# NVIDIA/RAD-MMM

Hardware: AMD Instinct MI355X
Metric: mel-frames/sec training step (fwd+bwd) (higher is better)
Workload: dtype f32 (f16 hi.hi product + fp8 e4m3 cross terms, fp32 accumulate); 1 GPU; RADTTS flow decoder (configs/RADTTS_model_config.yaml: 8 flows, WN 1024x4, D=1048) fwd+NLL+bwd; batch_per_gpu=32, n_mel=80, frames=800, global_batch=32, parallelism=dp1, includes_optimizer=False

## Files before the change

include/radmmm_hip.h:

```cpp
#ifndef RADMMM_HIP_H
#define RADMMM_HIP_H

#include <stdint.h>

#ifdef __cplusplus
extern "C" {
#endif

#define RADMMM_ABI_VERSION 4

typedef void* radmmm_stream_t;

const char* radmmm_last_error(void);
int radmmm_abi_version(void);

enum { RADMMM_ACT_NONE = 0, RADMMM_ACT_SOFTPLUS = 1, RADMMM_ACT_RELU = 2, RADMMM_ACT_LEAKY = 3 };
enum { RADMMM_SCALE_TANH = 0, RADMMM_SCALE_EXP = 1, RADMMM_SCALE_SIGMOID = 2, RADMMM_SCALE_TRANSLATE = 3 };

#define RADMMM_SPLIT_F16 0
#define RADMMM_SPLIT_X8A 1
#define RADMMM_SPLIT_X8B 2
typedef struct { int fmt; int x8_exp; int32_t* sat_flag;
                 void* lo16;
} radmmm_split_opts;
// ... 71 lines not shown
#define RADMMM_F32_FAMILY_WGRAD16 5
#define RADMMM_F32_KERNEL_CODE(family, bl, mt, rows) ((family) * 1000000 + (bl) * 100000 + (mt) * 1000 + (rows))
int radmmm_rowgemm_f32_plan(const radmmm_rowgemm_desc* d);
int radmmm_wgrad_f32_plan(const radmmm_wgrad_desc* d);

int radmmm_weightnorm_fwd(const float* v, const float* g, float* W, float* inv_norm,
                          int Cout, int Cin, int taps, int ldw,
                          int perm_split, int off_lo, int off_hi, radmmm_stream_t stream);
int radmmm_weightnorm_bwd(const float* v, const float* g, const float* inv_norm,
                          const float* dW, int splits, int64_t split_stride,
                          float* dv, float* dg,
                          int Cout, int Cin, int taps, int ldw,
                          int perm_split, int off_lo, int off_hi,
                          const float* poison ,
                          radmmm_stream_t stream);

int radmmm_wn_input_fwd(const float* ctx, int ldctx, const float* z, int ldz,
                        float* X0 , int ldx0, int rows, int D, int h,
                        void* X0h, void* X0l ,
                        const radmmm_split_opts* so, radmmm_stream_t stream);
int radmmm_wn_input_bwd(const float* gX0, int ldx0, float* gctx, int ldctx, int ctx_accum,
                        float* gz, int ldz, int rows, int D, int h, radmmm_stream_t stream);

int radmmm_squeeze_rows(const float* in , float* out, int B, int C, int T, int g, int ld, int col0,
                        radmmm_stream_t stream);
int radmmm_unsqueeze_rows(const float* gout, float* gin , int B, int C, int T, int g, int ld, int col0,
                          radmmm_stream_t stream);

int radmmm_affine_coupling_fwd(const float* O, int ldo, const float* z, int ldz,
                               float* zout, float* log_s, int rows, int h, int scaling,
// ... 144 lines not shown
int radmmm_wgrad_rm8(const void* GYh, const void* GYx, int ldg, int g8_exp, const void* Xh, const void* Xx, int ldx, int x8_exp,
                     int R, int T, const int32_t* lens, int x_mask, float* P, int ldp, int64_t split_stride, int Mc, int Nc,
                     int taps, int dil, int splits, float acc_scale, radmmm_stream_t stream);

int radmmm_wgrad_rmh(const void* GYh, int ldg, const void* Xh, int ldx, int R, int T, const int32_t* lens, int x_mask, float* P,
                     int ldp, int64_t split_stride, int Mc, int Nc, int taps, int dil, int splits, float acc_scale,
                     radmmm_stream_t stream);

int radmmm_wgrad_rmh_shift(const void* GYh, int ldg, int g_col0, const void* Xh, int ldx, int x_col0, int shift0, int R, int T,
                           const int32_t* lens, int x_mask, float* P, int ldp, int64_t split_stride, int Mc, int Nc, int taps,
                           int dil, int splits, float acc_scale, radmmm_stream_t stream);
int radmmm_wgrad_rm_shift(const void* GYh, const void* GYl, int ldg, int g_col0, const void* Xh, const void* Xl, int ldx, int x_col0,
                          int shift0, int R, int T, const int32_t* lens, int x_mask, float* P, int ldp, int64_t split_stride,
                          int Mc, int Nc, int taps, int dil, int splits, float acc_scale, radmmm_stream_t stream);

int radmmm_split_f16_groups(const float* x, int ld, void* hi, void* lo, int ldh, int rows, int gcols, int groups, int gpitch,
                            float scale, int* sat_flag, radmmm_stream_t stream);

int64_t radmmm_lstm_scratch_bytes(int B, int H, int which);
int64_t radmmm_lstm_hseq_bytes(int B, int T, int H);
int radmmm_lstm_fwd(float* G, const float* W_hh, float* y, float* c, const int32_t* lens, void* wsplit, void* hsplit,
                    void* hseq, int B, int T, int H, radmmm_stream_t stream);
int radmmm_lstm_bwd(float* G, const float* c, const float* dy, const float* W_hh, const int32_t* lens, void* wtpack,
                    float* P, float* dcbuf, int B, int T, int H, const float* gscale, radmmm_stream_t stream);
int radmmm_lstm_last_path(int which);

int radmmm_lu_weight_fwd(const float* P, const float* lower, const float* lower_diag, const float* upper,
                         const float* upper_diag, int c, float* W, int ldw, int col_offset, float* logdet,
                         radmmm_stream_t stream);
int radmmm_lu_weight_bwd(const float* P, const float* lower, const float* lower_diag, const float* upper,
// ... 135 lines not shown
```

rad_mmm_amd/_lib.py:

```python
from __future__ import annotations

import ctypes as C
import os
from typing import Optional

import torch

_HERE = os.path.dirname(os.path.abspath(__file__))
LIB_PATH = os.environ.get("RADMMM_LIB_PATH") or os.path.join(_HERE, "libradmmm_hip.so")



def debug_env(name: str, default: Optional[str] = None) -> Optional[str]:
    if os.environ.get("RADMMM_DEBUG", "0") in ("", "0"):
        return default
    return os.environ.get(name, default)


ACT_NONE, ACT_SOFTPLUS, ACT_RELU, ACT_LEAKY = 0, 1, 2, 3
SCALE = {"tanh": 0, "exp": 1, "sigmoid": 2, "translate": 3}
ACT = {"none": 0, "softplus": 1, "relu": 2, "leaky_relu": 3}


class RadmmmError(RuntimeError):
# ... 24 lines not shown
        ("split_fmt", C.c_int), ("ch_x8_exp", C.c_int), ("c2h_x8_exp", C.c_int),
        ("sat_flag", C.c_void_p),
        ("Clo", C.c_void_p),
        ("colsum_out", C.c_void_p), ("colsum_scratch", C.c_void_p),
        ("dact_h", C.c_void_p), ("dact_x", C.c_void_p), ("lddact_h", C.c_int), ("dact_x8_exp", C.c_int),
        ("c2_src", C.c_void_p * 3), ("n_c2_src", C.c_int),
    ]


class CsItem(C.Structure):
    _fields_ = [("part", C.c_void_p), ("out", C.c_void_p), ("nparts", C.c_int), ("cols", C.c_int)]


class DactItem(C.Structure):
    _fields_ = [("saved", C.c_void_p), ("yh", C.c_void_p), ("yl", C.c_void_p), ("ylo16", C.c_void_p), ("part", C.c_void_p)]


class SplitOpts(C.Structure):
    _fields_ = [("fmt", C.c_int), ("x8_exp", C.c_int), ("sat_flag", C.c_void_p), ("lo16", C.c_void_p)]


SPLIT_F16, SPLIT_X8A, SPLIT_X8B = 0, 1, 2


def split_opts(fmt: int = 0, x8_exp: int = 0, sat_flag: Optional[torch.Tensor] = None, lo16: Optional[torch.Tensor] = None):
    return C.byref(SplitOpts(fmt, x8_exp, sat_flag.data_ptr() if sat_flag is not None else None,
                             lo16.data_ptr() if lo16 is not None else None))


class RowGemmH3Desc(C.Structure):
# ... 65 lines not shown
        "radmmm_masked_reduce": [p, i, i, i, i64, i64, i64, p, i, p, p, p],
        "radmmm_masked_reduce_bwd": [p, i, i, i, i64, i64, i64, p, i, p, p, p],
        "radmmm_fused_add_tanh_sigmoid_multiply": [p, p, i, p, i, i, i, p],
        "radmmm_film_fwd": [p, i, p, i, p, i, p, p, p, p, p, i, i, i, i, p],
        "radmmm_film_bwd": [p, i, p, i, p, i, p, p, p, p, f, i, p, p, i, p, i, p, i, p, p, p, i, i, i, p],
        "radmmm_film_bwd_sums": [p, i, p, i, p, i, p, p, p, p, p, p, p, i, i, p],
        "radmmm_film_bwd_apply": [p, i, p, i, p, i, p, p, p, p, f, i, p, p, i, p, i, p, i, p, i, i, p],
        "radmmm_split_f16": [p, i, p, p, i, i, i, f, so, p],
        "radmmm_transpose_split_act": [p, i, i, i, i, i, i, p, i, f, p, p, p, p, i, p],
        "radmmm_wgrad_h3_tiles": [i, i, i],
        "radmmm_wgrad_rm_tiles": [i, i, i],
        "radmmm_wgrad_rm": [p, p, i, p, p, i, i, i, p, i, p, i, i64, i, i, i, i, i, f, p],
        "radmmm_wgrad_rm8": [p, p, i, i, p, p, i, i, i, i, p, i, p, i, i64, i, i, i, i, i, f, p],
        "radmmm_wgrad_rmh": [p, i, p, i, i, i, p, i, p, i, i64, i, i, i, i, i, f, p],
        "radmmm_wgrad_rmh_shift": [p, i, i, p, i, i, i, i, i, p, i, p, i, i64, i, i, i, i, i, f, p],
        "radmmm_wgrad_rm_shift": [p, p, i, i, p, p, i, i, i, i, i, p, i, p, i, i64, i, i, i, i, i, f, p],
        "radmmm_split_f16_groups": [p, i, p, p, i, i, i, i, i, f, p, p],
        "radmmm_betabinom_prior": [i, i, C.c_double, p, p],
        "radmmm_prior_zoom_batch": [p, i, p, i, i, p],
        "radmmm_energy_average": [p, p, i, i, i, i, p],
        "radmmm_lu_weight_fwd": [p, p, p, p, p, i, p, i, i, p, p],
        "radmmm_lu_weight_bwd": [p, p, p, p, p, i, p, i, i, p, p, p, p, p],
        "radmmm_instnorm_fwd": [p, i, p, p, p, i, p, p, p, i, i, i, f, i, p],
        "radmmm_instnorm_bwd": [p, i, p, i, p, i, p, p, p, p, i, p, p, p, i, i, i, i, p],
        "radmmm_pq_spline_inv": [p, i, p, i, p, i, i, i, i, p],
        "radmmm_sumsq": [p, i64, p, p],
        "radmmm_radam_step": [p, p, p, p, i64, p, f, f, f, f, f, i, p],
        "radmmm_transpose_split_act_colsum": [p, i, i, i, i, i, i, p, i, f, p, p, p, p, i, p, i, i, i, p],
        "radmmm_colsum_final": [p, p, i, i, p],
        "radmmm_colsum_final_multi": [C.POINTER(CsItem), i, p], "radmmm_rowgemm_h3_colsum_rows": [C.POINTER(RowGemmH3Desc)],
# ... 258 lines not shown
```

rad_mmm_amd/csrc/elementwise.hip:

```cpp
#include <math.h>
#include <stdlib.h>

#include "common.h"
#include "split_pack.h"

namespace {

using radmmm::block_sum;
using radmmm::wave_sum;

__device__ __forceinline__ int perm_col(int ci, int perm_split, int off_lo, int off_hi) {
  return ci < perm_split ? ci + off_lo : ci - perm_split + off_hi;
}

__global__ __launch_bounds__(256) void weightnorm_fwd_kernel(
    const float* __restrict__ v, const float* __restrict__ g, float* __restrict__ W,
    float* __restrict__ inv_norm, int Cout, int Cin, int taps, int ldw, int perm_split,
    int off_lo, int off_hi) {
  __shared__ float sh[17];
  const int co = blockIdx.x;
  const int n = Cin * taps;
  const float* vr = v + (long long)co * n;
  float ss = 0.f;
  for (int i = threadIdx.x; i < n; i += blockDim.x) ss = fmaf(vr[i], vr[i], ss);
// ... 77 lines not shown
  if (threadIdx.x == 0) dg[co] = dot * inv + (poison ? poison[0] : 0.f);
  const float a = gg * inv, b = gg * dot * inv * inv * inv;
  if (VEC && n % 4 == 0) {
    for (int i = threadIdx.x * 4; i < n; i += blockDim.x * 4) {
      const float4 vv = *reinterpret_cast<const float4*>(vr + i);
      const float4 gv = *reinterpret_cast<const float4*>(gw + i);
      *reinterpret_cast<float4*>(dv + (long long)co * n + i) =
          make_float4(a * gv.x - b * vv.x, a * gv.y - b * vv.y, a * gv.z - b * vv.z, a * gv.w - b * vv.w);
    }
  } else {
    for (int i = threadIdx.x; i < n; i += blockDim.x) dv[(long long)co * n + i] = a * gw[i] - b * vr[i];
  }
}

template <int TAPS>
__global__ __launch_bounds__(256) void weightnorm_bwd_reg_kernel(
    const float* __restrict__ v, const float* __restrict__ g, const float* __restrict__ inv_norm,
    const float* __restrict__ dW, int splits, long long split_stride, float* __restrict__ dv,
    float* __restrict__ dg, int Cout, int Cin, int ldw, int perm_split, int off_lo, int off_hi,
    const float* __restrict__ poison) {
  __shared__ float sh[17];
  const int co = blockIdx.x;
  const long long n = (long long)Cin * TAPS;
  const float inv = inv_norm[co], gg = g[co], pz = poison ? poison[0] : 0.f;
  constexpr int MAXJ = 2;
  float4 vv[MAXJ][TAPS], gs[MAXJ][TAPS];
  float dot = 0.f;
#pragma unroll
  for (int j = 0; j < MAXJ; ++j) {
    const int ci = threadIdx.x * 4 + j * 1024;
    const bool on = ci < Cin;
    const int cic = on ? ci : 0;
    const int col = perm_col(cic, perm_split, off_lo, off_hi);
    const float* vp = v + (long long)co * n + (long long)cic * TAPS;
#pragma unroll
    for (int k = 0; k < TAPS; ++k) vv[j][k] = on ? *reinterpret_cast<const float4*>(vp + 4 * k) : make_float4(0.f, 0.f, 0.f, 0.f);
#pragma unroll
// ... 23 lines not shown
  const float a = gg * inv, b = gg * dot * inv * inv * inv;
#pragma unroll
  for (int j = 0; j < MAXJ; ++j) {
    const int ci = threadIdx.x * 4 + j * 1024;
    if (ci < Cin) {
      float o[4 * TAPS];
#pragma unroll
      for (int c = 0; c < 4; ++c)
#pragma unroll
        for (int k = 0; k < TAPS; ++k) o[c * TAPS + k] = a * chan_of(gs[j][k], c) - b * run_at(vv[j], c * TAPS + k);
      float* dp = dv + (long long)co * n + (long long)ci * TAPS;
#pragma unroll
      for (int k = 0; k < TAPS; ++k) *reinterpret_cast<float4*>(dp + 4 * k) = make_float4(o[4 * k], o[4 * k + 1], o[4 * k + 2], o[4 * k + 3]);
    }
  }
}

__global__ __launch_bounds__(256) void wn_input_fwd_kernel(
    const float* __restrict__ ctx, int ldctx, const float* __restrict__ z, int ldz,
    float* __restrict__ X0, int ldx0, int rows, int D, int h, _Float16* __restrict__ Xh,
    _Float16* __restrict__ Xl, int fmt, float x8_mul, void* __restrict__ lo16) {
  const long long total = (long long)rows * ldx0;
  for (long long i = blockIdx.x * (long long)blockDim.x + threadIdx.x; i < total;
       i += (long long)gridDim.x * blockDim.x) {
    const int r = (int)(i / ldx0), c = (int)(i - (long long)r * ldx0);
    float v = 0.f;
    if (c < D) v = ctx[(long long)r * ldctx + c];
    else if (c < D + h) v = z[(long long)r * ldz + (c - D)];
    if (X0) X0[i] = v;
    if (Xh) radmmm::store_split1_fmt(Xh, Xl, (long long)r * ldx0, c, fmt, x8_mul, 1.f, v, lo16);
// ... 381 lines not shown
                           (long long)split_stride, dv, dg, Cout, Cin, ldw, perm_split, off_lo, off_hi, poison);
    } else if (vec)
      hipLaunchKernelGGL(weightnorm_bwd_lds_kernel<true>, dim3(Cout), dim3(256), lds, ST(stream), v, g, inv_norm, dW,
                         splits, (long long)split_stride, dv, dg, Cout, Cin, taps, ldw, perm_split, off_lo, off_hi, poison);
    else
      hipLaunchKernelGGL(weightnorm_bwd_lds_kernel<false>, dim3(Cout), dim3(256), lds, ST(stream), v, g, inv_norm, dW,
                         splits, (long long)split_stride, dv, dg, Cout, Cin, taps, ldw, perm_split, off_lo, off_hi, poison);
  } else {
    hipLaunchKernelGGL(weightnorm_bwd_kernel, dim3(Cout), dim3(256), 0, ST(stream), v, g, inv_norm, dW,
                       splits, (long long)split_stride, dv, dg, Cout, Cin, taps, ldw, perm_split,
                       off_lo, off_hi, poison);
  }
  return radmmm::check_launch("weightnorm_bwd");
}

extern "C" int radmmm_wn_input_fwd(const float* ctx, int ldctx, const float* z, int ldz, float* X0,
                                   int ldx0, int rows, int D, int h, void* Xh, void* Xl,
                                   const radmmm_split_opts* so, radmmm_stream_t stream) {
  RADMMM_REQUIRE(ctx && z && (X0 || Xh), "wn_input_fwd: null pointer (X0 may be NULL when the split copy Xh / Xl is written)");
  RADMMM_REQUIRE(rows > 0 && D > 0 && h > 0 && ldx0 >= D + h && ldctx >= D && ldz >= h, "wn_input_fwd: bad dims");
  const int fmt = so ? so->fmt : RADMMM_SPLIT_F16;
  RADMMM_REQUIRE(fmt == RADMMM_SPLIT_F16 || !Xh || (ldx0 % 32 == 0 && abs(so->x8_exp) <= 16), "wn_input_fwd: 8-bit format needs ldx0 %% 32 == 0");
  auto a16 = [](const void* q) { return (reinterpret_cast<uintptr_t>(q) & 15) == 0; };
  auto a8 = [](const void* q) { return (reinterpret_cast<uintptr_t>(q) & 7) == 0; };
  if (D % 4 == 0 && ldctx % 4 == 0 && ldz % 4 == 0 && ldx0 % 4 == 0 && a16(ctx) && a16(z) && a16(X0) &&
      a8(Xh) && a8(Xl) && a8(so ? so->lo16 : nullptr)) {
    hipLaunchKernelGGL(wn_input_fwd4_kernel, dim3(grid_for((long long)rows * (ldx0 / 4))), dim3(256), 0, ST(stream), ctx,
                       ldctx, z, ldz, X0, ldx0, rows, D, h, static_cast<_Float16*>(Xh), static_cast<_Float16*>(Xl), fmt,
                       ldexpf(1.f, so ? so->x8_exp : 0), so ? so->lo16 : nullptr);
    return radmmm::check_launch("wn_input_fwd");
// ... 245 lines not shown
```

rad_mmm_amd/csrc/wgrad_rm8.hip:

```cpp
#include <cstdlib>
#include <type_traits>

#include "common.h"

namespace {

typedef float f32x16 __attribute__((ext_vector_type(16)));
typedef _Float16 f16x8 __attribute__((ext_vector_type(8)));
typedef _Float16 f16x2 __attribute__((ext_vector_type(2)));
typedef short i16x2 __attribute__((ext_vector_type(2)));
typedef int i32x2 __attribute__((ext_vector_type(2)));
typedef int i32x4 __attribute__((ext_vector_type(4)));
typedef int i32x8 __attribute__((ext_vector_type(8)));
typedef __attribute__((address_space(3))) unsigned int* lds_u32_ptr;

constexpr int BK = 32, TM = 256, TN = 256;
constexpr int HARR = BK * TM * 2;
constexpr int LARR = BK * TM;
constexpr int NSTAGE = 3;
constexpr int stage_bytes(int PR) { return 2 * HARR + (PR == 2 ? 2 * LARR : 0); }
constexpr int HH_NSTAGE = 3;
constexpr int smem_bytes(int PR) { return (PR == 2 ? NSTAGE : HH_NSTAGE) * stage_bytes(PR); }
constexpr int OOB = 0x7fffffff;

// ... 147 lines not shown
      if (i == 1) nmask = row_mask();
      if (i == 7) frag_issue<8192>(xb1[0], bh_base[0] + sbn);
      __builtin_amdgcn_sched_barrier(0);
      acc[i][1] = __builtin_amdgcn_mfma_f32_32x32x16_f16(ah1, bh1[1], acc[i][1], 0, 0, 0);
      __builtin_amdgcn_sched_barrier(0);
      if (i < 4) dma_piece(nbuf, 2 * i + 1, l_rel, nmask);
      if (i == 7) frag_issue<8192>(xb1[1], bh_base[1] + sbn);
      __builtin_amdgcn_sched_barrier(0);
    }
    buf = xbuf;
  }
  asm volatile("s_waitcnt vmcnt(0) lgkmcnt(0)" ::: "memory");
  __syncthreads();
}

template <int PR>
__global__ __launch_bounds__(256, 1) void wgrad_rm8_kernel(const Rm8Args a) {
  extern __shared__ __attribute__((aligned(16))) unsigned char sm[];
  constexpr int STAGE = stage_bytes(PR);
  constexpr int NPIECE = PR == 2 ? 12 : 8;
  if constexpr (PR == 2) asm volatile("s_setreg_imm32_b32 hwreg(HW_REG_MODE, 23, 1), 1");
  const int tid = threadIdx.x, lane = tid & 63;
  const int wave = __builtin_amdgcn_readfirstlane(tid >> 6);
  const int ntm = (a.Mc + TM - 1) / TM, ntn = (a.Nc + TN - 1) / TN;
  const int nt = ntm * ntn * a.taps * a.splits, wg = blockIdx.x;
  const int xcd = wg & 7, loc = wg >> 3, qq = nt >> 3, r8 = nt & 7;
  int id = (xcd < r8 ? xcd * (qq + 1) : r8 * (qq + 1) + (xcd - r8) * qq) + loc;
  const int tn = id % ntn; id /= ntn;
  const int tm = id % ntm; id /= ntm;
  const int tap = id % a.taps;
  const int split = id / a.taps;
  const int m0 = tm * TM, n0 = tn * TN;
  const int shift = (tap - a.taps / 2) * a.dil + a.shift0;
  const int steps_total = (a.R + BK - 1) / BK;
  const int steps_per = (steps_total + a.splits - 1) / a.splits;
  const int step_lo = split * steps_per;
  int step_hi = step_lo + steps_per;
  if (step_hi > steps_total) step_hi = steps_total;
  const int nsteps = step_hi - step_lo;

  const __amdgpu_buffer_rsrc_t rGh = __builtin_amdgcn_make_buffer_rsrc(const_cast<_Float16*>(a.GYh), 0, a.g_bytes, 0x00020000);
  const __amdgpu_buffer_rsrc_t rXh = __builtin_amdgcn_make_buffer_rsrc(const_cast<_Float16*>(a.Xh), 0, a.x_bytes, 0x00020000);
// ... 217 lines not shown
    __syncthreads();
  }
  float* P = a.P + (long long)split * a.split_stride + (long long)tap * a.Mc * a.ldp;
  {
    const int colb = n0 + wave * 64 + (lane & 31);
#pragma unroll
    for (int I = 0; I < 8; ++I)
#pragma unroll
      for (int j = 0; j < 2; ++j)
#pragma unroll
        for (int e = 0; e < 16; ++e) {
          const int row = m0 + I * 32 + (e & 3) + 8 * (e >> 2) + 4 * (lane >> 5), col = colb + j * 32;
          if (row < a.Mc && col < a.Nc) P[(long long)row * a.ldp + col] = acc[I][j][e] * a.acc_scale;
        }
  }
}

}

extern "C" int radmmm_wgrad_rm8(const void* GYh, const void* GYx, int ldg, int g8_exp, const void* Xh, const void* Xx, int ldx,
                                int x8_exp, int R, int T, const int32_t* lens, int x_mask, float* P, int ldp, int64_t split_stride,
                                int Mc, int Nc, int taps, int dil, int splits, float acc_scale, radmmm_stream_t stream) {
  RADMMM_REQUIRE(GYh && GYx && Xh && Xx && P, "wgrad_rm8: null pointer");
  RADMMM_REQUIRE(Mc > 0 && Nc > 0 && taps >= 1 && dil >= 1 && splits >= 1 && R > 0 && T > 0 && R % T == 0 && ldg >= Mc &&
                     ldx >= Nc && ldg % 32 == 0 && ldx % 32 == 0 && ldp >= Nc && T >= BK && R / T <= 1024 &&
                     abs(g8_exp) <= 16 && abs(x8_exp) <= 16,
                 "wgrad_rm8: bad dims (ldg, ldx %% 32 == 0, R = B * T, T >= 32, B <= 1024, |x8_exp| <= 16)");
  RADMMM_REQUIRE(radmmm::aligned16(GYh) && radmmm::aligned16(GYx) && radmmm::aligned16(Xh) && radmmm::aligned16(Xx),
                 "wgrad_rm8: 16-byte aligned operands");
  const long long g_bytes = (long long)R * ldg * 2, x_bytes = (long long)R * ldx * 2;
// ... 15 lines not shown
  a.xl_pitch = 2 * ldx; a.xl_bstride = 64; a.xl_boff = 32;
  a.g8_exp = g8_exp; a.x8_exp = x8_exp;
  a.lens = lens; a.x_mask = x_mask;
  a.R = R; a.T = T; a.ldg = ldg; a.ldx = ldx; a.Mc = Mc; a.Nc = Nc; a.taps = taps; a.dil = dil; a.splits = splits;
  a.P = P; a.ldp = ldp; a.split_stride = split_stride; a.acc_scale = acc_scale;
  a.g_bytes = (int)g_bytes; a.x_bytes = (int)x_bytes; a.gl_bytes = (int)g_bytes; a.xl_bytes = (int)x_bytes;
  a.g_col0 = 0; a.x_col0 = 0; a.shift0 = 0;
  const int tiles = ((Mc + TM - 1) / TM) * ((Nc + TN - 1) / TN) * taps;
  hipLaunchKernelGGL(wgrad_rm8_kernel<2>, dim3(tiles * splits), dim3(256), smem_bytes(2) + 4096, static_cast<hipStream_t>(stream), a);
  return radmmm::check_launch("wgrad_rm8");
}


namespace {

int launch_rmh(const char* who, const void* GYh, int ldg, int g_col0, const void* Xh, int ldx, int x_col0, int shift0, int R, int T,
               const int32_t* lens, int x_mask, float* P, int ldp, int64_t split_stride, int Mc, int Nc, int taps, int dil,
               int splits, float acc_scale, radmmm_stream_t stream) {
  RADMMM_REQUIRE(GYh && Xh && P, "%s: null pointer", who);
  RADMMM_REQUIRE(Mc > 0 && Nc > 0 && taps >= 1 && dil >= 1 && splits >= 1 && R > 0 && T > 0 && R % T == 0 && ldg >= Mc &&
                     ldx >= Nc && ldg % 32 == 0 && ldx % 32 == 0 && ldp >= Nc && T >= BK && R / T <= 1024,
                 "%s: bad dims (ldg, ldx %% 32 == 0, R = B * T, T >= 32, B <= 1024, splits >= 1)", who);
  RADMMM_REQUIRE(g_col0 >= 0 && x_col0 >= 0 && g_col0 % 8 == 0 && x_col0 % 8 == 0 && (long long)g_col0 + Mc <= ldg &&
                     (long long)x_col0 + Nc <= ldx,
                 "%s: bad column origin (multiples of 8, g_col0 + Mc <= ldg, x_col0 + Nc <= ldx)", who);
  RADMMM_REQUIRE(radmmm::wgrad_rm_shift_fits(R, ldx, shift0, taps, dil),
                 "%s: shift0 out of range ((R + 96 + |shift0| + (taps / 2) * dil) * ldx * 2 must stay below 2^31)", who);
  RADMMM_REQUIRE(radmmm::aligned16(GYh) && radmmm::aligned16(Xh), "%s: 16-byte aligned operands", who);
  const long long g_bytes = (long long)R * ldg * 2, x_bytes = (long long)R * ldx * 2;
  RADMMM_REQUIRE(g_bytes < 0x7fffffffLL && x_bytes < 0x7fffffffLL, "%s: operand >= 2 GiB", who);
  static int once = [] {
    hipError_t e = hipFuncSetAttribute(reinterpret_cast<const void*>(wgrad_rm8_kernel<1>), hipFuncAttributeMaxDynamicSharedMemorySize,
                                       smem_bytes(1) + 4096);
    if (e != hipSuccess) {
      radmmm::set_error("hipFuncSetAttribute(wgrad_rmh): %s", hipGetErrorString(e));
      return -2;
    }
    return 0;
  }();
  if (once) return once;
  Rm8Args a = {};
  a.GYh = static_cast<const _Float16*>(GYh); a.Xh = static_cast<const _Float16*>(Xh);
  a.lens = lens; a.x_mask = x_mask;
  a.R = R; a.T = T; a.ldg = ldg; a.ldx = ldx; a.Mc = Mc; a.Nc = Nc; a.taps = taps; a.dil = dil; a.splits = splits;
  a.P = P; a.ldp = ldp; a.split_stride = split_stride; a.acc_scale = acc_scale;
// ... 7 lines not shown
}

extern "C" int radmmm_wgrad_rmh(const void* GYh, int ldg, const void* Xh, int ldx, int R, int T, const int32_t* lens, int x_mask,
                                float* P, int ldp, int64_t split_stride, int Mc, int Nc, int taps, int dil, int splits,
                                float acc_scale, radmmm_stream_t stream) {
  return launch_rmh("wgrad_rmh", GYh, ldg, 0, Xh, ldx, 0, 0, R, T, lens, x_mask, P, ldp, split_stride, Mc, Nc, taps, dil, splits,
                    acc_scale, stream);
}

extern "C" int radmmm_wgrad_rmh_shift(const void* GYh, int ldg, int g_col0, const void* Xh, int ldx, int x_col0, int shift0, int R,
                                      int T, const int32_t* lens, int x_mask, float* P, int ldp, int64_t split_stride, int Mc,
                                      int Nc, int taps, int dil, int splits, float acc_scale, radmmm_stream_t stream) {
  return launch_rmh("wgrad_rmh_shift", GYh, ldg, g_col0, Xh, ldx, x_col0, shift0, R, T, lens, x_mask, P, ldp, split_stride, Mc, Nc,
                    taps, dil, splits, acc_scale, stream);
}
```

rad_mmm_amd/ops.py:

```python
from __future__ import annotations

import collections
import math
import os
import types
from typing import List, Optional, Sequence, Tuple

import torch

from . import _lib as L
from ._lib import (ACT, SCALE, lib, check, ptr, stream, rowgemm, wgrad, f32c, amp_fwd, amp_bwd, split_opts, SPLIT_F16,
                   SPLIT_X8A, SPLIT_X8B)

ZLD = 160


def _empty(*shape, like: torch.Tensor) -> torch.Tensor:
    return torch.empty(*shape, device=like.device, dtype=torch.float32)


def round_up(x: int, m: int) -> int:
    return (x + m - 1) // m * m


# ... 780 lines not shown
          "wgrad_rm8")
    return P


def wgrad_rmh_slabs(gh, xh, B, T, Mc, Nc, taps, dil, acc_scale, lens=None):
    R = B * T
    assert gh.shape[0] >= R and xh.shape[0] >= R and gh.dtype == torch.float16 and xh.dtype == torch.float16
    tiles = int(lib.radmmm_wgrad_rm_tiles(Mc, Nc, taps))
    S = pick_splits(tiles, R, slots=int(lib.radmmm_gemm_cu_slots()))
    P = torch.empty(S, taps, Mc, Nc, device=gh.device, dtype=torch.float32)
    assert gh.stride(1) == 1 and xh.stride(1) == 1
    check(lib.radmmm_wgrad_rmh(ptr(gh), gh.stride(0), ptr(xh), xh.stride(0), R, T, ptr(lens), 1 if lens is not None else 0,
                               ptr(P), Nc, P.stride(0), Mc, Nc, taps, dil, S, acc_scale, stream()),
          "wgrad_rmh")
    return P


def split_f16_groups(x, gcols, groups, scale=1.0, gpitch=None, with_lo=True, sat_flag=None):
    rows = x.shape[0]
    gpitch = gpitch or round_up(gcols, 32)
    ldh = groups * gpitch
    assert x.dim() == 2 and x.stride(1) == 1 and x.dtype == torch.float32
    hi = torch.empty(rows, ldh, device=x.device, dtype=torch.float16)
    lo = torch.empty(rows, ldh, device=x.device, dtype=torch.float16) if with_lo else None
    check(lib.radmmm_split_f16_groups(ptr(x), x.stride(0), ptr(hi), ptr(lo), ldh, rows, gcols, groups, gpitch, scale,
                                      ptr(sat_flag), stream()), "split_f16_groups")
    return hi, lo


def wgrad_rm_shift_slabs(gy_pair, g_col0, x_pair, x_col0, shift0, B, T, Mc, Nc, acc_scale, lens=None):
# ... 543 lines not shown
            if rows > 0:
                batch.add(kw["colsum_scratch"], gb, rows, kw["N"])
        pair_h = pair_l = None
        WT_prev = None
        x_prev = None
        multi = bool(use_rm and 2 <= nl <= 4 and act and debug_env("RADMMM_DACT_MULTI", "1") != "0")
        pre_pairs, gq_pre = {}, None
        if multi:
            for j in range(nl - 1, 0, -1):
                pre_pairs[j] = _halves(2 * N, Wc, like=z_in)
            top = _halves(N, Wc, like=z_in)
            gq_dst = [(pre_pairs[j + 1][0][N:], pre_pairs[j + 1][1][N:]) if j < nl - 1 else top for j in range(nl)]
            gq_sums = dact_mul_rows_multi(gOUT, [R[j] for j in range(nl)], Wc, B, T, act, SG, gq_dst, [None] * nl, fa, GE, flag,
                                          [grad_out(res_p[3 * j + 2]) for j in range(nl)], defer=batch)
            gq_pre = (gq_dst, gq_sums)
        for j in range(nl - 1, -1, -1):
            d = 2 ** j
            kt = in_p[3 * j].shape[2]
            fused = pair_h is not None
            if gq_pre is not None:
                (gQh, gQl), g_res[3 * j + 2] = gq_pre[0][j], gq_pre[1][j]
                gy_t = None
            else:
                if fused:
                    gQh, gQl = pair_h[N:], pair_l[N:]
                else:
                    gQh, gQl = _halves(N, Wc, like=z_in)
                gy_t, g_res[3 * j + 2] = dact_mul_transposed(gOUT, R[j], Wc, B, T, act, SG, None if use_rm else "gy", gQh, gQl, fa,
                                                             GE, flag, sum_out=grad_out(res_p[3 * j + 2]), defer=batch)
            if use_rm:
                slabs = wg_rm((gQh, gQl), Hpair[j + 1], Wc, Wc, 1, 1)
            else:
                x_t = x_prev if x_prev is not None else transpose_split_act(H[j + 1], Wc, B, T, None, 0, 1.0, "x")
                slabs = wgrad_h3_slabs(gy_t, x_t, Wc, Wc, Wc, 1, 1, 1.0 / SG, WPR)
            g_res[3 * j], g_res[3 * j + 1] = weightnorm_bwd(res_p[3 * j], res_p[3 * j + 1], inv_r[j], slabs, Wc, poison=poison)
            keep_pair = j > 0
            nh, nlo = pre_pairs[j] if (keep_pair and j in pre_pairs) else _halves(2 * N if keep_pair else N, Wc, like=z_in)
            gch, gcl = nh[:N], nlo[:N]
            g_conv = None if pair_only else _empty(N, Wc, like=z_in)
            if pair_only:
                dsrc = dict(dact_h=Hpair[j + 1][0], dact_x=Hpair[j + 1][1], lddact_h=Wc, dact_x8_exp=X8_ACT_EXP)
            else:
                dsrc = dict(dact_src=H[j + 1], lddact=Wc)
            epi = dict(C=g_conv, ldc=Wc, M=N, N=Wc, K=Wc, lens=lens, dact=act, **dsrc,
                       rowscale=2 if partial else 1, ratio_taps=kt, ratio_dil=d, Ch=gch, Cl=gcl, ldch=Wc, ch_scale=SG)
            gb, cs = cs_args(in_p[3 * j + 2])
            if fused:
                WTh, WTl, ktn, dn = WT_prev
                if pre is None:
                    transpose_split(Wrh[j], Wrl[j], Wc, Wc, Wc, NPR, out=(WTh[ktn:], WTl[ktn:]))
# ... 184 lines not shown
```

Before: 708,800 mel-frames/s.

## Group residual wgrad GEMMs and weightnorm backward across WN layers into single launches

Adds grouped kernels that fold the per-layer 1x1 residual weight-gradient GEMMs (f16 row-major path) into one launch, with a job table and XCD-aware tile mapping. A matching multi-item weightnorm backward kernel covers all layers' residual weights at once. The goal is to cut launch overhead and fill the GPU better than several small serial GEMMs. The cost is computing all slabs up front, which uses more temporary memory, and the path only runs when the multi-dact, pair-only and single-product conditions hold.

```diff
diff --git a/include/radmmm_hip.h b/include/radmmm_hip.h
--- a/include/radmmm_hip.h
+++ b/include/radmmm_hip.h
@@ -109,6 +109,19 @@
                           int perm_split, int off_lo, int off_hi,
                           const float* poison ,
                           radmmm_stream_t stream);
+typedef struct radmmm_wnb_item {
+  const float* v;
+  const float* g;
+  const float* inv_norm;
+  const float* dW;
+  float* dv;
+  float* dg;
+  int64_t split_stride;
+  int splits;
+  int Cout, Cin, ldw;
+  int perm_split, off_lo, off_hi;
+} radmmm_wnb_item;
+int radmmm_weightnorm_bwd_multi(const radmmm_wnb_item* items, int n, int taps, const float* poison, radmmm_stream_t stream);
 
 int radmmm_wn_input_fwd(const float* ctx, int ldctx, const float* z, int ldz,
                         float* X0 , int ldx0, int rows, int D, int h,
@@ -283,6 +296,19 @@
                           int shift0, int R, int T, const int32_t* lens, int x_mask, float* P, int ldp, int64_t split_stride,
                           int Mc, int Nc, int taps, int dil, int splits, float acc_scale, radmmm_stream_t stream);
 
+typedef struct radmmm_wg_item {
+  const void* GYh;
+  const void* Xh;
+  float* P;
+  int64_t split_stride;
+  int ldg, g_col0;
+  int ldx, x_col0;
+  int Mc, Nc;
+  int ldp;
+} radmmm_wg_item;
+int radmmm_wgrad_rmh_group(const radmmm_wg_item* items, int n, int shift0, int R, int T, const int32_t* lens, int x_mask, int taps,
+                           int dil, int splits, float acc_scale, radmmm_stream_t stream);
+
 int radmmm_split_f16_groups(const float* x, int ld, void* hi, void* lo, int ldh, int rows, int gcols, int groups, int gpitch,
                             float scale, int* sat_flag, radmmm_stream_t stream);
 
diff --git a/rad_mmm_amd/_lib.py b/rad_mmm_amd/_lib.py
--- a/rad_mmm_amd/_lib.py
+++ b/rad_mmm_amd/_lib.py
@@ -62,6 +62,18 @@
 
 class DactItem(C.Structure):
     _fields_ = [("saved", C.c_void_p), ("yh", C.c_void_p), ("yl", C.c_void_p), ("ylo16", C.c_void_p), ("part", C.c_void_p)]
+
+
+class WgItem(C.Structure):
+    _fields_ = [("GYh", C.c_void_p), ("Xh", C.c_void_p), ("P", C.c_void_p), ("split_stride", C.c_int64),
+                ("ldg", C.c_int), ("g_col0", C.c_int), ("ldx", C.c_int), ("x_col0", C.c_int), ("Mc", C.c_int), ("Nc", C.c_int),
+                ("ldp", C.c_int)]
+
+
+class WnbItem(C.Structure):
+    _fields_ = [("v", C.c_void_p), ("g", C.c_void_p), ("inv_norm", C.c_void_p), ("dW", C.c_void_p), ("dv", C.c_void_p),
+                ("dg", C.c_void_p), ("split_stride", C.c_int64), ("splits", C.c_int), ("Cout", C.c_int), ("Cin", C.c_int),
+                ("ldw", C.c_int), ("perm_split", C.c_int), ("off_lo", C.c_int), ("off_hi", C.c_int)]
 
 
 class SplitOpts(C.Structure):
@@ -157,6 +169,8 @@
         "radmmm_wgrad_rm8": [p, p, i, i, p, p, i, i, i, i, p, i, p, i, i64, i, i, i, i, i, f, p],
         "radmmm_wgrad_rmh": [p, i, p, i, i, i, p, i, p, i, i64, i, i, i, i, i, f, p],
         "radmmm_wgrad_rmh_shift": [p, i, i, p, i, i, i, i, i, p, i, p, i, i64, i, i, i, i, i, f, p],
+        "radmmm_wgrad_rmh_group": [C.POINTER(WgItem), i, i, i, i, p, i, i, i, i, f, p],
+        "radmmm_weightnorm_bwd_multi": [C.POINTER(WnbItem), i, i, p, p],
         "radmmm_wgrad_rm_shift": [p, p, i, i, p, p, i, i, i, i, i, p, i, p, i, i64, i, i, i, i, i, f, p],
         "radmmm_split_f16_groups": [p, i, p, p, i, i, i, i, i, f, p, p],
         "radmmm_betabinom_prior": [i, i, C.c_double, p, p],
diff --git a/rad_mmm_amd/csrc/elementwise.hip b/rad_mmm_amd/csrc/elementwise.hip
--- a/rad_mmm_amd/csrc/elementwise.hip
+++ b/rad_mmm_amd/csrc/elementwise.hip
@@ -115,13 +115,12 @@
 }
 
 template <int TAPS>
-__global__ __launch_bounds__(256) void weightnorm_bwd_reg_kernel(
+__device__ __forceinline__ void weightnorm_bwd_reg_row(
     const float* __restrict__ v, const float* __restrict__ g, const float* __restrict__ inv_norm,
     const float* __restrict__ dW, int splits, long long split_stride, float* __restrict__ dv,
     float* __restrict__ dg, int Cout, int Cin, int ldw, int perm_split, int off_lo, int off_hi,
-    const float* __restrict__ poison) {
+    const float* __restrict__ poison, int co) {
   __shared__ float sh[17];
-  const int co = blockIdx.x;
   const long long n = (long long)Cin * TAPS;
   const float inv = inv_norm[co], gg = g[co], pz = poison ? poison[0] : 0.f;
   constexpr int MAXJ = 2;
@@ -175,6 +174,33 @@
       for (int k = 0; k < TAPS; ++k) *reinterpret_cast<float4*>(dp + 4 * k) = make_float4(o[4 * k], o[4 * k + 1], o[4 * k + 2], o[4 * k + 3]);
     }
   }
+}
+
+template <int TAPS>
+__global__ __launch_bounds__(256) void weightnorm_bwd_reg_kernel(
+    const float* __restrict__ v, const float* __restrict__ g, const float* __restrict__ inv_norm,
+    const float* __restrict__ dW, int splits, long long split_stride, float* __restrict__ dv,
+    float* __restrict__ dg, int Cout, int Cin, int ldw, int perm_split, int off_lo, int off_hi,
+    const float* __restrict__ poison) {
+  weightnorm_bwd_reg_row<TAPS>(v, g, inv_norm, dW, splits, split_stride, dv, dg, Cout, Cin, ldw, perm_split, off_lo, off_hi, poison, blockIdx.x);
+}
+
+constexpr int WNB_MAX = 8;
+struct WnbGroup {
+  radmmm_wnb_item it[WNB_MAX];
+  int first[WNB_MAX + 1];
+  const float* poison;
+};
+template <int TAPS>
+__global__ __launch_bounds__(256) void weightnorm_bwd_multi_kernel(const WnbGroup m) {
+  const int b = blockIdx.x;
+  int k = 0;
+#pragma unroll
+  for (int q = 1; q < WNB_MAX; ++q) k += b >= m.first[q] ? 1 : 0;
+  k = __builtin_amdgcn_readfirstlane(k);
+  const radmmm_wnb_item& t = m.it[k];
+  weightnorm_bwd_reg_row<TAPS>(t.v, t.g, t.inv_norm, t.dW, t.splits, (long long)t.split_stride, t.dv, t.dg, t.Cout, t.Cin, t.ldw,
+                               t.perm_split, t.off_lo, t.off_hi, m.poison, b - m.first[k]);
 }
 
 __global__ __launch_bounds__(256) void wn_input_fwd_kernel(
@@ -586,6 +612,32 @@
   return radmmm::check_launch("weightnorm_bwd");
 }
 
+extern "C" int radmmm_weightnorm_bwd_multi(const radmmm_wnb_item* items, int n, int taps, const float* poison,
+                                           radmmm_stream_t stream) {
+  RADMMM_REQUIRE(items, "weightnorm_bwd_multi: null items");
+  RADMMM_REQUIRE(n >= 1 && n <= WNB_MAX, "weightnorm_bwd_multi: n=%d items (1 .. %d)", n, WNB_MAX);
+  RADMMM_REQUIRE(taps == 1, "weightnorm_bwd_multi: taps=%d (one-tap tensors only)", taps);
+  WnbGroup m = {};
+  long long total = 0;
+  auto a16 = [](const void* q) { return (reinterpret_cast<uintptr_t>(q) & 15) == 0; };
+  for (int k = 0; k < n; ++k) {
+    const radmmm_wnb_item& t = items[k];
+    RADMMM_REQUIRE(t.v && t.g && t.inv_norm && t.dW && t.dv && t.dg, "weightnorm_bwd_multi: null pointer (item %d)", k);
+    RADMMM_REQUIRE(t.Cout > 0 && t.Cin > 0 && t.ldw >= t.Cin && t.splits >= 1, "weightnorm_bwd_multi: bad dims (item %d)", k);
+    RADMMM_REQUIRE(t.Cin % 4 == 0 && t.Cin <= 2048 && t.perm_split % 4 == 0 && t.off_lo % 4 == 0 && t.off_hi % 4 == 0 &&
+                       t.ldw % 4 == 0 && t.split_stride % 4 == 0 && a16(t.dW) && a16(t.v) && a16(t.dv),
+                   "weightnorm_bwd_multi: item %d is not on the register path (Cin %% 4 == 0, Cin <= 2048, 16-byte conditions)", k);
+    m.it[k] = t;
+    m.first[k] = (int)total;
+    total += t.Cout;
+    RADMMM_REQUIRE(total < 0x7fffffffLL, "weightnorm_bwd_multi: too many output channels");
+  }
+  for (int k = n; k <= WNB_MAX; ++k) m.first[k] = (int)total;
+  m.poison = poison;
+  hipLaunchKernelGGL(weightnorm_bwd_multi_kernel<1>, dim3((unsigned)total), dim3(256), 0, ST(stream), m);
+  return radmmm::check_launch("weightnorm_bwd_multi");
+}
+
 extern "C" int radmmm_wn_input_fwd(const float* ctx, int ldctx, const float* z, int ldz, float* X0,
                                    int ldx0, int rows, int D, int h, void* Xh, void* Xl,
                                    const radmmm_split_opts* so, radmmm_stream_t stream) {
diff --git a/rad_mmm_amd/csrc/wgrad_rm8.hip b/rad_mmm_amd/csrc/wgrad_rm8.hip
--- a/rad_mmm_amd/csrc/wgrad_rm8.hip
+++ b/rad_mmm_amd/csrc/wgrad_rm8.hip
@@ -185,8 +185,13 @@
   __syncthreads();
 }
 
+__device__ __forceinline__ int xcd_tile_id(int nt, int wg) {
+  const int xcd = wg & 7, loc = wg >> 3, qq = nt >> 3, r8 = nt & 7;
+  return (xcd < r8 ? xcd * (qq + 1) : r8 * (qq + 1) + (xcd - r8) * qq) + loc;
+}
+
 template <int PR>
-__global__ __launch_bounds__(256, 1) void wgrad_rm8_kernel(const Rm8Args a) {
+__device__ __forceinline__ void wgrad_rm8_tile(const Rm8Args& a, int id) {
   extern __shared__ __attribute__((aligned(16))) unsigned char sm[];
   constexpr int STAGE = stage_bytes(PR);
   constexpr int NPIECE = PR == 2 ? 12 : 8;
@@ -194,9 +199,6 @@
   const int tid = threadIdx.x, lane = tid & 63;
   const int wave = __builtin_amdgcn_readfirstlane(tid >> 6);
   const int ntm = (a.Mc + TM - 1) / TM, ntn = (a.Nc + TN - 1) / TN;
-  const int nt = ntm * ntn * a.taps * a.splits, wg = blockIdx.x;
-  const int xcd = wg & 7, loc = wg >> 3, qq = nt >> 3, r8 = nt & 7;
-  int id = (xcd < r8 ? xcd * (qq + 1) : r8 * (qq + 1) + (xcd - r8) * qq) + loc;
   const int tn = id % ntn; id /= ntn;
   const int tm = id % ntm; id /= ntm;
   const int tap = id % a.taps;
@@ -444,6 +446,44 @@
           if (row < a.Mc && col < a.Nc) P[(long long)row * a.ldp + col] = acc[I][j][e] * a.acc_scale;
         }
   }
+}
+
+template <int PR>
+__global__ __launch_bounds__(256, 1) void wgrad_rm8_kernel(const Rm8Args a) {
+  const int nt = ((a.Mc + TM - 1) / TM) * ((a.Nc + TN - 1) / TN) * a.taps * a.splits;
+  wgrad_rm8_tile<PR>(a, xcd_tile_id(nt, blockIdx.x));
+}
+
+constexpr int WG_MAX = 8;
+struct Rm8Job {
+  const _Float16 *GYh, *Xh;
+  float* P;
+  long long split_stride;
+  int ldg, ldx, Mc, Nc, ldp, g_bytes, x_bytes, g_col0, x_col0;
+};
+struct Rm8Group {
+  Rm8Job job[WG_MAX];
+  int first[WG_MAX + 1];
+  const int* lens;
+  int x_mask, R, T, taps, dil, splits, shift0;
+  float acc_scale;
+};
+
+__global__ __launch_bounds__(256, 1) void wgrad_rmh_group_kernel(const Rm8Group g) {
+  const int id = xcd_tile_id(g.first[WG_MAX], blockIdx.x);
+  int k = 0;
+#pragma unroll
+  for (int q = 1; q < WG_MAX; ++q) k += id >= g.first[q] ? 1 : 0;
+  k = __builtin_amdgcn_readfirstlane(k);
+  const Rm8Job& jb = g.job[k];
+  Rm8Args a = {};
+  a.GYh = jb.GYh; a.Xh = jb.Xh;
+  a.lens = g.lens; a.x_mask = g.x_mask;
+  a.R = g.R; a.T = g.T; a.ldg = jb.ldg; a.ldx = jb.ldx; a.Mc = jb.Mc; a.Nc = jb.Nc; a.taps = g.taps; a.dil = g.dil; a.splits = g.splits;
+  a.P = jb.P; a.ldp = jb.ldp; a.split_stride = jb.split_stride; a.acc_scale = g.acc_scale;
+  a.g_bytes = jb.g_bytes; a.x_bytes = jb.x_bytes;
+  a.g_col0 = jb.g_col0; a.x_col0 = jb.x_col0; a.shift0 = g.shift0;
+  wgrad_rm8_tile<1>(a, id - g.first[k]);
 }
 
 }
@@ -489,9 +529,8 @@
 
 namespace {
 
-int launch_rmh(const char* who, const void* GYh, int ldg, int g_col0, const void* Xh, int ldx, int x_col0, int shift0, int R, int T,
-               const int32_t* lens, int x_mask, float* P, int ldp, int64_t split_stride, int Mc, int Nc, int taps, int dil,
-               int splits, float acc_scale, radmmm_stream_t stream) {
+int check_rmh(const char* who, const void* GYh, int ldg, int g_col0, const void* Xh, int ldx, int x_col0, int shift0, int R, int T,
+              const float* P, int ldp, int Mc, int Nc, int taps, int dil, int splits) {
   RADMMM_REQUIRE(GYh && Xh && P, "%s: null pointer", who);
   RADMMM_REQUIRE(Mc > 0 && Nc > 0 && taps >= 1 && dil >= 1 && splits >= 1 && R > 0 && T > 0 && R % T == 0 && ldg >= Mc &&
                      ldx >= Nc && ldg % 32 == 0 && ldx % 32 == 0 && ldp >= Nc && T >= BK && R / T <= 1024,
@@ -504,6 +543,14 @@
   RADMMM_REQUIRE(radmmm::aligned16(GYh) && radmmm::aligned16(Xh), "%s: 16-byte aligned operands", who);
   const long long g_bytes = (long long)R * ldg * 2, x_bytes = (long long)R * ldx * 2;
   RADMMM_REQUIRE(g_bytes < 0x7fffffffLL && x_bytes < 0x7fffffffLL, "%s: operand >= 2 GiB", who);
+  return 0;
+}
+
+int launch_rmh(const char* who, const void* GYh, int ldg, int g_col0, const void* Xh, int ldx, int x_col0, int shift0, int R, int T,
+               const int32_t* lens, int x_mask, float* P, int ldp, int64_t split_stride, int Mc, int Nc, int taps, int dil,
+               int splits, float acc_scale, radmmm_stream_t stream) {
+  if (const int bad = check_rmh(who, GYh, ldg, g_col0, Xh, ldx, x_col0, shift0, R, T, P, ldp, Mc, Nc, taps, dil, splits)) return bad;
+  const long long g_bytes = (long long)R * ldg * 2, x_bytes = (long long)R * ldx * 2;
   static int once = [] {
     hipError_t e = hipFuncSetAttribute(reinterpret_cast<const void*>(wgrad_rm8_kernel<1>), hipFuncAttributeMaxDynamicSharedMemorySize,
                                        smem_bytes(1) + 4096);
@@ -541,3 +588,42 @@
   return launch_rmh("wgrad_rmh_shift", GYh, ldg, g_col0, Xh, ldx, x_col0, shift0, R, T, lens, x_mask, P, ldp, split_stride, Mc, Nc,
                     taps, dil, splits, acc_scale, stream);
 }
+
+extern "C" int radmmm_wgrad_rmh_group(const radmmm_wg_item* items, int n, int shift0, int R, int T, const int32_t* lens, int x_mask,
+                                      int taps, int dil, int splits, float acc_scale, radmmm_stream_t stream) {
+  RADMMM_REQUIRE(items, "wgrad_rmh_group: null items");
+  RADMMM_REQUIRE(n >= 1 && n <= WG_MAX, "wgrad_rmh_group: n=%d jobs (1 .. %d)", n, WG_MAX);
+  Rm8Group g = {};
+  long long total = 0;
+  for (int k = 0; k < n; ++k) {
+    const radmmm_wg_item& t = items[k];
+    if (const int bad = check_rmh("wgrad_rmh_group", t.GYh, t.ldg, t.g_col0, t.Xh, t.ldx, t.x_col0, shift0, R, T, t.P, t.ldp, t.Mc,
+                                  t.Nc, taps, dil, splits))
+      return bad;
+    Rm8Job& jb = g.job[k];
+    jb.GYh = static_cast<const _Float16*>(t.GYh); jb.Xh = static_cast<const _Float16*>(t.Xh);
+    jb.P = t.P; jb.split_stride = t.split_stride;
+    jb.ldg = t.ldg; jb.ldx = t.ldx; jb.Mc = t.Mc; jb.Nc = t.Nc; jb.ldp = t.ldp;
+    jb.g_bytes = (int)((long long)R * t.ldg * 2); jb.x_bytes = (int)((long long)R * t.ldx * 2);
+    jb.g_col0 = t.g_col0; jb.x_col0 = t.x_col0;
+    g.first[k] = (int)total;
+    total += (long long)((t.Mc + TM - 1) / TM) * ((t.Nc + TN - 1) / TN) * taps * splits;
+    RADMMM_REQUIRE(total < 0x7fffffffLL, "wgrad_rmh_group: too many workgroups");
+  }
+  for (int k = n; k <= WG_MAX; ++k) g.first[k] = (int)total;
+  g.lens = lens; g.x_mask = x_mask;
+  g.R = R; g.T = T; g.taps = taps; g.dil = dil; g.splits = splits; g.shift0 = shift0;
+  g.acc_scale = acc_scale;
+  static int once = [] {
+    hipError_t e = hipFuncSetAttribute(reinterpret_cast<const void*>(wgrad_rmh_group_kernel), hipFuncAttributeMaxDynamicSharedMemorySize,
+                                       smem_bytes(1) + 4096);
+    if (e != hipSuccess) {
+      radmmm::set_error("hipFuncSetAttribute(wgrad_rmh_group): %s", hipGetErrorString(e));
+      return -2;
+    }
+    return 0;
+  }();
+  if (once) return once;
+  hipLaunchKernelGGL(wgrad_rmh_group_kernel, dim3((unsigned)total), dim3(256), smem_bytes(1) + 4096, static_cast<hipStream_t>(stream), g);
+  return radmmm::check_launch("wgrad_rmh_group");
+}
diff --git a/rad_mmm_amd/ops.py b/rad_mmm_amd/ops.py
--- a/rad_mmm_amd/ops.py
+++ b/rad_mmm_amd/ops.py
@@ -818,6 +818,38 @@
                                ptr(P), Nc, P.stride(0), Mc, Nc, taps, dil, S, acc_scale, stream()),
           "wgrad_rmh")
     return P
+
+
+def wgrad_rmh_group_slabs(jobs, B, T, taps, dil, acc_scale, lens=None, splits=None, shift0=0):
+    R = B * T
+    jobs = [tuple(j) + (0, 0) * (len(j) == 4) for j in jobs]
+    for gh, xh, Mc, Nc, g0, x0 in jobs:
+        assert gh.shape[0] >= R and xh.shape[0] >= R and gh.dtype == torch.float16 and xh.dtype == torch.float16
+        assert gh.stride(1) == 1 and xh.stride(1) == 1
+    tiles = sum(int(lib.radmmm_wgrad_rm_tiles(Mc, Nc, taps)) for _, _, Mc, Nc, _, _ in jobs)
+    S = splits or pick_splits(tiles, R, slots=int(lib.radmmm_gemm_cu_slots()))
+    Ps = [torch.empty(S, taps, Mc, Nc, device=gh.device, dtype=torch.float32) for gh, _, Mc, Nc, _, _ in jobs]
+    items = (L.WgItem * len(jobs))(*[L.WgItem(ptr(gh), ptr(xh), ptr(P), P.stride(0), gh.stride(0), g0, xh.stride(0), x0, Mc, Nc, Nc)
+                                     for (gh, xh, Mc, Nc, g0, x0), P in zip(jobs, Ps)])
+    check(lib.radmmm_wgrad_rmh_group(items, len(jobs), shift0, R, T, ptr(lens), 1 if lens is not None else 0, taps, dil, S,
+                                     acc_scale, stream()), "wgrad_rmh_group")
+    return Ps
+
+
+def weightnorm_bwd_multi(vs, gs, invs, slabs, ldw: int, poison: Optional[torch.Tensor] = None):
+    dvs, dgs = [grad_out(v) for v in vs], [grad_out(g) for g in gs]
+    items = (L.WnbItem * len(vs))(*[L.WnbItem(ptr(v), ptr(g), ptr(inv), ptr(P), ptr(dv), ptr(dg), P.stride(0), P.shape[0],
+                                              v.shape[0], v.shape[1], ldw, 0, 0, 0)
+                                    for v, g, inv, P, dv, dg in zip(vs, gs, invs, slabs, dvs, dgs)])
+    one_tap = all(v.shape[2] == 1 for v in vs)
+    rc = lib.radmmm_weightnorm_bwd_multi(items, len(vs), 1, ptr(poison), stream()) if one_tap else -1
+    if not one_tap or (rc == -1 and b"register path" in lib.radmmm_last_error()):
+        for v, g, inv, P, dv, dg in zip(vs, gs, invs, slabs, dvs, dgs):
+            check(lib.radmmm_weightnorm_bwd(ptr(v), ptr(g), ptr(inv), ptr(P), P.shape[0], P.stride(0), ptr(dv), ptr(dg), v.shape[0],
+                                            v.shape[1], v.shape[2], ldw, 0, 0, 0, ptr(poison), stream()), "weightnorm_bwd")
+    else:
+        check(rc, "weightnorm_bwd_multi")
+    return list(zip(dvs, dgs))
 
 
 def split_f16_groups(x, gcols, groups, scale=1.0, gpitch=None, with_lo=True, sat_flag=None):
@@ -1391,6 +1423,14 @@
             gq_sums = dact_mul_rows_multi(gOUT, [R[j] for j in range(nl)], Wc, B, T, act, SG, gq_dst, [None] * nl, fa, GE, flag,
                                           [grad_out(res_p[3 * j + 2]) for j in range(nl)], defer=batch)
             gq_pre = (gq_dst, gq_sums)
+        grouped = bool(multi and pair_only and plan.wgrad_products == 1 and debug_env("RADMMM_WGRAD_GROUP", "1") != "0")
+        if grouped:
+            res_slabs = wgrad_rmh_group_slabs([(gq_dst[j][0], Hpair[j + 1][0], Wc, Wc) for j in range(nl)], B, T, 1, 1, 1.0 / SG)
+            res_g = weightnorm_bwd_multi([res_p[3 * j] for j in range(nl)], [res_p[3 * j + 1] for j in range(nl)],
+                                         [inv_r[j] for j in range(nl)], res_slabs, Wc, poison=poison)
+            for j in range(nl):
+                g_res[3 * j], g_res[3 * j + 1] = res_g[j]
+            del res_slabs
         for j in range(nl - 1, -1, -1):
             d = 2 ** j
             kt = in_p[3 * j].shape[2]
@@ -1405,12 +1445,15 @@
                     gQh, gQl = _halves(N, Wc, like=z_in)
                 gy_t, g_res[3 * j + 2] = dact_mul_transposed(gOUT, R[j], Wc, B, T, act, SG, None if use_rm else "gy", gQh, gQl, fa,
                                                              GE, flag, sum_out=grad_out(res_p[3 * j + 2]), defer=batch)
-            if use_rm:
+            if grouped:
+                slabs = None
+            elif use_rm:
                 slabs = wg_rm((gQh, gQl), Hpair[j + 1], Wc, Wc, 1, 1)
             else:
                 x_t = x_prev if x_prev is not None else transpose_split_act(H[j + 1], Wc, B, T, None, 0, 1.0, "x")
                 slabs = wgrad_h3_slabs(gy_t, x_t, Wc, Wc, Wc, 1, 1, 1.0 / SG, WPR)
-            g_res[3 * j], g_res[3 * j + 1] = weightnorm_bwd(res_p[3 * j], res_p[3 * j + 1], inv_r[j], slabs, Wc, poison=poison)
+            if not grouped:
+                g_res[3 * j], g_res[3 * j + 1] = weightnorm_bwd(res_p[3 * j], res_p[3 * j + 1], inv_r[j], slabs, Wc, poison=poison)
             keep_pair = j > 0
             nh, nlo = pre_pairs[j] if (keep_pair and j in pre_pairs) else _halves(2 * N if keep_pair else N, Wc, like=z_in)
             gch, gcl = nh[:N], nlo[:N]
```

Result: faster. 724,200 mel-frames/s (median of 6 runs) (+2.2%).
